# zhaihongjia/SplatLoc

Measured on AMD Instinct MI355X. Metric: fwd+bwd frames/s @1080p, 500k Gaussians, 32 feat-ch; HBM GB/s vs roofline, higher is better.
Workload: dtype f32

## Files before the change

include/splatraster.h:

```cpp
#ifndef SPLATRASTER_H
#define SPLATRASTER_H

#include <stddef.h>
#include <stdint.h>

#ifdef __cplusplus
extern "C" {
#endif

#define SPLATRASTER_ABI_VERSION 20

#define SPLATRASTER_TILE 16

#define SPLATRASTER_OK 0
#define SPLATRASTER_ERR_BAD_ARG 1
#define SPLATRASTER_ERR_HIP 2
#define SPLATRASTER_ERR_UNSUPPORTED 3
#define SPLATRASTER_ERR_OVERFLOW 4
#define SPLATRASTER_WARN_LOOKBACK_STALL 5

typedef struct splatraster_settings {
    int32_t image_height;
    int32_t image_width;
    float tanfovx;
// ... 482 lines not shown
#define SPLATRASTER_STAGE_PAYLOAD 9
#define SPLATRASTER_STAGE_COUNT 10

int splatraster_timing_enable(int on);
int splatraster_timing_select(uint32_t stage_mask);
int splatraster_timing_collect(double* ms, int64_t* counts);


int splatraster_poll_errors(void);
int splatraster_debug_set_spin_limit(uint32_t limit);
int splatraster_debug_set_deterministic(int on);
int splatraster_debug_set_small_panel_max_waves(int waves);
int splatraster_debug_set_split_max_waves(int waves);
int splatraster_debug_set_fwd_team(int mode);
int splatraster_debug_set_payload_stream_min(int64_t instances);
int splatraster_debug_set_front_end(int mode);
int splatraster_debug_set_tile_sort_cap(int keys);
int splatraster_debug_set_sort_fork(int mode);
int splatraster_debug_exp2(int64_t n, const float* x, float* y, void* stream);
int splatraster_debug_poison_lds(uint32_t pattern, void* stream);

const char* splatraster_error_string(int status);
const char* splatraster_last_hip_error(void);
int splatraster_abi_version(void);

#ifdef __cplusplus
}
#endif
#endif
```

splatloc_amd/_native.py:

```python
from __future__ import annotations

import ctypes as C
import os

from . import build as _build

_LIB = None
ABI_VERSION = 20

OK = 0
WARN_LOOKBACK_STALL = 5
_ERR_NAMES = {1: "bad argument", 2: "HIP runtime error", 3: "unsupported configuration",
              4: "tile instance count overflow", 5: "look-back stall (results late, never wrong)"}


class Settings(C.Structure):
    _fields_ = [
        ("image_height", C.c_int32),
        ("image_width", C.c_int32),
        ("tanfovx", C.c_float),
        ("tanfovy", C.c_float),
        ("scale_modifier", C.c_float),
        ("sh_degree", C.c_int32),
        ("sh_coeffs", C.c_int32),
# ... 112 lines not shown
                                            + [_vp] * 14),
    "splatraster_forward_window_geometry_raw": (C.c_int, [C.POINTER(Settings), _i32, C.POINTER(WindowView), _i32, _vp, C.POINTER(RawForward),
                                                          _vp, C.POINTER(_i64), _vp]),
    "splatraster_backward_window_raw": (C.c_int, [C.POINTER(Settings), _i32, C.POINTER(WindowView), _i32, C.POINTER(_i64)]
                                        + [_vp] * 8 + [C.POINTER(RawParams)] + [_vp] * 2),
    "splatraster_get_window_geometry_layout": (C.c_int, [_i32, _i32, C.POINTER(GeometryLayout)]),
    "splatraster_get_window_binning_layout": (C.c_int, [_i32, _i32, _i64, _i32, _i32, _i32, C.POINTER(BinningLayout)]),
    "splatraster_get_window_image_layout": (C.c_int, [_i32, _i32, _i32, C.POINTER(ImageLayout)]),
    "splatraster_debug_set_small_panel_max_waves": (C.c_int, [C.c_int]),
    "splatraster_debug_set_split_max_waves": (C.c_int, [C.c_int]),
    "splatraster_debug_set_fwd_team": (C.c_int, [C.c_int]),
    "splatraster_debug_set_front_end": (C.c_int, [C.c_int]),
    "splatraster_debug_set_tile_sort_cap": (C.c_int, [C.c_int]),
    "splatraster_debug_set_sort_fork": (C.c_int, [C.c_int]),
    "splatraster_debug_set_payload_stream_min": (C.c_int, [C.c_int64]),
    "splatraster_mark_visible": (C.c_int, [_i32, _vp, _vp, _vp, _vp, _vp]),
    "splatraster_get_geometry_layout": (C.c_int, [_i32, C.POINTER(GeometryLayout)]),
    "splatraster_get_binning_layout": (C.c_int, [_i32, _i64, _i32, _i32, _i32, C.POINTER(BinningLayout)]),
    "splatraster_get_image_layout": (C.c_int, [_i32, _i32, C.POINTER(ImageLayout)]),
    "splatraster_sort_tmp_bytes": (_sz, [_i64]),
    "splatraster_sort_pairs_u32": (C.c_int, [_i64, _vp, _vp, _i32, _vp, _vp]),
    "splatraster_timing_enable": (C.c_int, [C.c_int]),
    "splatraster_timing_select": (C.c_int, [C.c_uint32]),
    "splatraster_timing_collect": (C.c_int, [_vp, _vp]),
    "splatknn_workspace_bytes": (_sz, [_i32]),
    "splatknn_dist2": (C.c_int, [_i32, _vp, _vp, _vp, _vp]),
    "splatknn_debug_set_grid_min": (C.c_int, [_i32]),
    "splatraster_grid_encoding_layout": (C.c_int, [_i32] * 5 + [C.c_double, _i32, C.POINTER(GridLayout)]),
    "splatraster_grid_encoding_forward": (C.c_int, [C.POINTER(GridLayout), _i64, _vp, _vp, _vp, _vp]),
    "splatraster_grid_encoding_backward": (C.c_int, [C.POINTER(GridLayout), _i64] + [_vp] * 6),
# ... 84 lines not shown
    got = int(lib.splatraster_abi_version())
    if got != ABI_VERSION:
        raise RuntimeError(f"{path} has ABI version {got}, this binding needs {ABI_VERSION}: stale library, "
                           "rebuild with `python -m splatloc_amd.build --force`")
    for name, (res, args) in SYMBOLS.items():
        fn = getattr(lib, name)
        fn.restype = res
        fn.argtypes = args
    _LIB = lib
    if os.environ.get("SPLATRASTER_SPLIT_MAX_WAVES"):
        lib.splatraster_debug_set_split_max_waves(int(os.environ["SPLATRASTER_SPLIT_MAX_WAVES"]))
    if os.environ.get("SPLATRASTER_FWD_TEAM"):
        lib.splatraster_debug_set_fwd_team(int(os.environ["SPLATRASTER_FWD_TEAM"]))
    if os.environ.get("SPLATRASTER_FRONT_END"):
        lib.splatraster_debug_set_front_end(int(os.environ["SPLATRASTER_FRONT_END"]))
    if os.environ.get("SPLATRASTER_TILE_SORT_CAP"):
        lib.splatraster_debug_set_tile_sort_cap(int(os.environ["SPLATRASTER_TILE_SORT_CAP"]))
    if os.environ.get("SPLATRASTER_SORT_FORK"):
        lib.splatraster_debug_set_sort_fork(int(os.environ["SPLATRASTER_SORT_FORK"]))
    if os.environ.get("SPLATRASTER_SMALL_PANEL_MAX_WAVES"):
        lib.splatraster_debug_set_small_panel_max_waves(int(os.environ["SPLATRASTER_SMALL_PANEL_MAX_WAVES"]))
    return lib


def check(status: int, what: str) -> None:
    if status != OK:
        lib = load()
        detail = lib.splatraster_last_hip_error().decode() if status in (2, 5) else ""
        raise RuntimeError(f"{what} failed: {_ERR_NAMES.get(status, status)} {detail}".strip())

# ... 17 lines not shown
    n = len(STAGES)
    ms = (C.c_double * n)()
    cnt = (C.c_int64 * n)()
    check(load().splatraster_timing_collect(ms, cnt), "timing_collect")
    return {s: (ms[i], cnt[i]) for i, s in enumerate(STAGES)}


def set_deterministic(on: bool) -> None:
    check(load().splatraster_debug_set_deterministic(int(bool(on))), "set_deterministic")


def set_front_end(mode: int) -> None:
    check(load().splatraster_debug_set_front_end(int(mode)), "set_front_end")


def poll_stall() -> bool:
    st = load().splatraster_poll_errors()
    if st == WARN_LOOKBACK_STALL:
        return True
    check(st, "poll_errors")
    return False
```

splatloc_amd/csrc/binning.hip:

```cpp
#include "tile_order.h"
#include "composite_common.h"

namespace sr {

__device__ __forceinline__ int f2i_sat_b(float v)
{
    if (!(v > -1.0e9f)) v = -1.0e9f;
    if (!(v < 1.0e9f)) v = 1.0e9f;
    return (int)v;
}

constexpr int EMIT_BLOCK = 256;
constexpr int EMIT_IPT = 4;
static_assert(EMIT_SPAN == EMIT_BLOCK * EMIT_IPT, "common.h: EMIT_SPAN");

template <typename KeyT>
__global__ void __launch_bounds__(EMIT_BLOCK)
emit_kernel(int64_t R, int P , int Pv , int tiles_per_view, int W, int H,
            const uint32_t* __restrict__ offsets,
            const uint32_t* __restrict__ depth_order, const float4* __restrict__ rec,
            KeyT* __restrict__ keys, uint32_t* __restrict__ vals,
            const uint32_t* __restrict__ span_owner ,
            uint32_t* __restrict__ ranges, uint32_t nranges )
{
// ... 135 lines not shown

int launch_payload(const splatraster_settings& s, int32_t V, int64_t R, const GeomView& g, const BinView& b, hipStream_t stream)
{
    if (R == 0) return SPLATRASTER_OK;
    const int gx = (s.image_width + TILE - 1) / TILE, gy = (s.image_height + TILE - 1) / TILE;
    if (R >= g_payload_stream_min)
        hipLaunchKernelGGL(payload_kernel<true>, dim3((unsigned)((R + 255) / 256)), dim3(256), 0, stream, R, gx, gx * gy, V,
                           b.point_list, b.tile_list, g.rec, b.irec, b.ipack, b.ranges);
    else
        hipLaunchKernelGGL(payload_kernel<false>, dim3((unsigned)((R + 255) / 256)), dim3(256), 0, stream, R, gx, gx * gy, V,
                           b.point_list, b.tile_list, g.rec, b.irec, b.ipack, b.ranges);
    SR_LAUNCH_CHECK();
    return SPLATRASTER_OK;
}

__global__ void __launch_bounds__(ORDER_THREADS)
tile_order_kernel(int T, const uint32_t* __restrict__ ranges, uint32_t* __restrict__ order, uint32_t* __restrict__ nparts)
{
    __shared__ uint32_t s_cnt[ORDER_BUCKETS];
    __shared__ uint32_t s_wsum[ORDER_THREADS / WAVE];
    tile_order_block(T, [&](int i) { return ranges[2 * i + 1] - ranges[2 * i]; }, order, s_cnt, s_wsum, nparts);
}

int launch_tile_order(const splatraster_settings& s, int32_t V, const BinView& b, hipStream_t stream)
{
    const int gx = (s.image_width + TILE - 1) / TILE, gy = (s.image_height + TILE - 1) / TILE;
    if (!use_tile_order(V, gx * gy)) return SPLATRASTER_OK;
    hipLaunchKernelGGL(tile_order_kernel, dim3(1), dim3(ORDER_THREADS), 0, stream, V * gx * gy, b.ranges, b.tile_order, b.nparts);
    SR_LAUNCH_CHECK();
    return SPLATRASTER_OK;
// ... 32 lines not shown
```

splatloc_amd/csrc/capi.hip:

```cpp
#include <string.h>

#include <mutex>
#include <unordered_map>
#include <string>
#include <vector>

#include "common.h"

namespace sr {

static thread_local std::string g_last_error;
static int g_deterministic = 0;
static int g_split_max_waves = SPLIT_MAX_WAVES;
void set_split_max_waves(int waves) { g_split_max_waves = waves < 0 ? SPLIT_MAX_WAVES : (waves > SPLIT_MAX_WAVES ? SPLIT_MAX_WAVES : waves); }
int split_max_waves() { return g_split_max_waves; }

void set_hip_error(hipError_t e, const char* what)
{
    g_last_error = std::string(what) + ": " + hipGetErrorString(e);
}

void set_error_text(const char* text) { g_last_error = text; }

struct StageRec { int stage; hipEvent_t a, b; };
// ... 169 lines not shown
    v.ipack = reinterpret_cast<uint32_t*>(b + L.ipack);
    v.featp = reinterpret_cast<float*>(b + L.featp);
    v.gacc = reinterpret_cast<float*>(b + L.gacc);
    v.pose_acc = reinterpret_cast<float*>(b + L.pose_acc);
    v.ckpt = reinterpret_cast<float*>(b + L.ckpt);
    v.tile_order = reinterpret_cast<uint32_t*>(b + L.tile_order);
    v.nparts = reinterpret_cast<uint32_t*>(b + L.nparts);
    return v;
}

static size_t img_plane_bytes(int32_t W, int32_t H, int32_t V)
{
    return align_up((size_t)W * H * 4 * (size_t)(V > 0 ? V : 1), 256);
}

ImgView img_view(void* base, int32_t W, int32_t H, int32_t V)
{
    char* b = reinterpret_cast<char*>(base);
    ImgView v;
    v.final_T = reinterpret_cast<float*>(b);
    v.n_contrib = reinterpret_cast<uint32_t*>(b + img_plane_bytes(W, H, V));
    return v;
}

static int check_row_index_range(int32_t P, int32_t V, int32_t C)
{
    const uint64_t n = (uint64_t)P * (uint64_t)V;
    if (n > (1ull << 24) || n * (uint64_t)padded_channels(C) >= (1ull << 32)) return SPLATRASTER_ERR_UNSUPPORTED;
    if ((uint64_t)gacc_total_floats(C, (size_t)P, (size_t)V) >= (1ull << 32)) return SPLATRASTER_ERR_UNSUPPORTED;
    return SPLATRASTER_OK;
}

static int check_settings(const splatraster_settings* s)
{
    if (!s) return SPLATRASTER_ERR_BAD_ARG;
    if (s->image_width <= 0 || s->image_height <= 0 || s->channels <= 0) return SPLATRASTER_ERR_BAD_ARG;
// ... 17 lines not shown
        case SPLATRASTER_ERR_HIP: return "HIP runtime error";
        case SPLATRASTER_ERR_UNSUPPORTED: return "unsupported configuration";
        case SPLATRASTER_ERR_OVERFLOW: return "tile instance count overflow";
        case SPLATRASTER_WARN_LOOKBACK_STALL: return "look-back stall (results late, never wrong)";
        default: return "unknown status";
    }
}

const char* splatraster_last_hip_error(void) { return g_last_error.c_str(); }

size_t splatraster_geometry_bytes(int32_t P) { return geom_layout(P, 1).bytes; }
size_t splatraster_binning_bytes(int32_t P, int64_t R, int32_t width, int32_t height, int32_t channels)
{
    return bin_layout(P, 1, R, width, height, channels).bytes;
}
size_t splatraster_image_bytes(int32_t width, int32_t height) { return 2 * img_plane_bytes(width, height, 1); }

size_t splatraster_window_geometry_bytes(int32_t P, int32_t n_views) { return geom_layout(P, n_views).bytes; }
size_t splatraster_window_binning_bytes(int32_t P, int32_t n_views, int64_t R_total, int32_t width, int32_t height,
                                        int32_t channels)
{
    return bin_layout(P, n_views, R_total, width, height, channels).bytes;
}
size_t splatraster_window_image_bytes(int32_t width, int32_t height, int32_t n_views)
{
    return 2 * img_plane_bytes(width, height, n_views);
}

int splatraster_get_geometry_layout(int32_t P, splatraster_geometry_layout* out)
{
    return splatraster_get_window_geometry_layout(P, 1, out);
}
int splatraster_get_window_geometry_layout(int32_t P, int32_t n_views, splatraster_geometry_layout* out)
{
    if (!out || n_views < 1 || n_views > MAX_VIEWS) return SPLATRASTER_ERR_BAD_ARG;
    const GeomLayout L = geom_layout(P, n_views);
    out->rec0 = L.rec0; out->rec1 = L.rec1; out->tiles_touched = L.tiles_touched;
    out->depth_order = L.depth_order; out->offsets = L.offsets; out->rgb = L.rgb;
    out->clamped = L.clamped; out->total = L.bytes;
    return SPLATRASTER_OK;
}
// ... 7 lines not shown
{
    if (!out || n_views < 1 || n_views > MAX_VIEWS) return SPLATRASTER_ERR_BAD_ARG;
    const BinLayout L = bin_layout(P, n_views, R_total, width, height, channels);
    out->point_list = L.valsA; out->tile_list = L.keysA; out->ranges = L.ranges; out->total = L.bytes;
    return SPLATRASTER_OK;
}
int splatraster_get_image_layout(int32_t width, int32_t height, splatraster_image_layout* out)
{
    return splatraster_get_window_image_layout(width, height, 1, out);
}
int splatraster_get_window_image_layout(int32_t width, int32_t height, int32_t n_views, splatraster_image_layout* out)
{
    if (!out || n_views < 1 || n_views > MAX_VIEWS) return SPLATRASTER_ERR_BAD_ARG;
    out->final_T = 0;
    out->n_contrib = img_plane_bytes(width, height, n_views);
    out->total = 2 * img_plane_bytes(width, height, n_views);
    return SPLATRASTER_OK;
}

}

namespace sr {

static int check_window(const splatraster_settings* s, int32_t V, const splatraster_window_view* views)
{
    int st = check_settings(s);
    if (st) return st;
    if (V < 1 || V > MAX_VIEWS || !views) return SPLATRASTER_ERR_BAD_ARG;
    return SPLATRASTER_OK;
}

// ... 14 lines not shown
struct BinScratch { bool on; uint32_t* table; void* scan_tmp; int64_t entries; };

static std::mutex g_front_end_mu;
static std::unordered_map<const void*, bool> g_front_end;
static void front_end_record(const void* geometry, bool on)
{
    std::lock_guard<std::mutex> lk(g_front_end_mu);
    if (g_front_end.size() > (1u << 14)) g_front_end.clear();
    g_front_end[geometry] = on;
}
static int front_end_recorded(const void* geometry)
{
    std::lock_guard<std::mutex> lk(g_front_end_mu);
    auto it = g_front_end.find(geometry);
    return it == g_front_end.end() ? -1 : (it->second ? 1 : 0);
}

static BinScratch bin_scratch(const splatraster_settings& s, int32_t P, int32_t V, void* geometry, bool geometry_stage)
{
    const int gx = (s.image_width + TILE - 1) / TILE, gy = (s.image_height + TILE - 1) / TILE, tiles = gx * gy;
    const GeomLayout L = geom_layout(P, V);
    BinScratch b{};
    if (!geometry || P <= 0) return b;
    const int recorded = geometry_stage ? -1 : front_end_recorded(geometry);
    b.on = recorded >= 0 ? recorded == 1 : use_bins(P, V, gx, gy, L.total - L.sort_keys);
    if (geometry_stage) front_end_record(geometry, b.on);
    if (!b.on) return b;
    char* base = reinterpret_cast<char*>(geometry);
    b.entries = (int64_t)bin_table_entries(P, V, tiles);
    b.table = reinterpret_cast<uint32_t*>(base + L.sort_keys);
// ... 143 lines not shown
        if (st) return st;
        bool in_alt = false;
        {
            StageTimer t(SPLATRASTER_STAGE_TILE_SORT, stream);
            st = keys16 ? sort_pairs_k16(R, k0, v0, k1, v1, bits, b.sort_tmp, stream, &in_alt)
                        : sort_pairs_u32(R, k0, v0, k1, v1, bits, b.sort_tmp, stream, &in_alt);
        }
        if (st) return st;
    }
    if (R == 0) {
        StageTimer t(SPLATRASTER_STAGE_RANGES, stream);
        st = launch_ranges_clear((int32_t)gtiles, b.ranges, stream);
    }
    if (st) return st;
    const float* featp = feat;
    if (R > 0) {
        StageTimer t(SPLATRASTER_STAGE_PAYLOAD, stream);
        if (!bins.on) st = launch_payload(*s, V, R, g, b, stream);
        if (st) return st;
        if (s->channels % 4) {
            st = launch_pad_features(P, s->channels, feat, b.featp, stream);
            featp = b.featp;
        }
    }
    if (st) return st;
    if (!(R > 0 && bins.on)) {
        StageTimer t(SPLATRASTER_STAGE_RANGES, stream);
        st = launch_tile_order(*s, V, b, stream);
    }
    if (st) return st;
    WinOut outs{};
    for (int v = 0; v < V; ++v) {
        outs.color[v] = views[v].out_color;
        outs.depth[v] = views[v].out_depth;
        outs.alpha[v] = views[v].out_alpha;
    }
    StageTimer t(SPLATRASTER_STAGE_COMPOSITE_FWD, stream);
    return launch_composite_fwd(*s, P, V, R, g, b, im, featp, bg, outs, stream);
}

struct BwdRows { GeomView g; BinView b; WinCams cams; WinGrad grads; };
static int window_accumulate(const splatraster_settings* s, int32_t V, const splatraster_window_view* views, int32_t P, int64_t R,
                             const float* bg, const float* colors_precomp, bool sh_colours, void* geometry, const void* binning,
                             const void* image, bool pose, hipStream_t stream, BwdRows* out)
{
    int st = check_row_index_range(P, V, s->channels);
    if (st) return st;
    const int W = s->image_width, H = s->image_height;
    GeomView& g = out->g;
    BinView& b = out->b;
    g = geom_view(geometry, P, V);
// ... 13 lines not shown
    }
    for (int v = 0; v < V; ++v) {
        const int gcv = views[v].color_grad_channels ? views[v].color_grad_channels : C;
        if (gcv != grads.gc) return SPLATRASTER_ERR_BAD_ARG;
        grads.dL_dlast[v] = grads.gc < C ? views[v].dL_dout_last : nullptr;
    }
    for (int v = 0; v < V; ++v) {
        grads.out_color[v] = views[v].out_color;
        grads.out_depth[v] = views[v].out_depth;
        grads.dL_dcolor[v] = views[v].dL_dout_color;
        grads.dL_ddepth[v] = views[v].dL_dout_depth;
        grads.dL_dalpha[v] = views[v].dL_dout_alpha;
        grads.dL_dmeans2D[v] = views[v].dL_dmeans2D;
    }
    const size_t gacc_n = gacc_total_floats(C, (size_t)P, (size_t)V);
    const bool det = g_deterministic != 0;
    long long* gacc64 = nullptr;
    if (det) {
        SR_HIP_CHECK(hipMallocAsync(reinterpret_cast<void**>(&gacc64), sizeof(long long) * gacc_n, stream));
        SR_HIP_CHECK(hipMemsetAsync(gacc64, 0, sizeof(long long) * gacc_n, stream));
    }
    const size_t fill = pose ? (size_t)(reinterpret_cast<char*>(b.pose_acc) - reinterpret_cast<char*>(b.gacc)) + POSE_ACC_BYTES
                             : sizeof(float) * gacc_n;
    SR_HIP_CHECK(hipMemsetAsync(b.gacc, 0, fill, stream));
    grads.bg = bg;
    grads.bg_channels = bg ? s->bg_channels : 0;
    {
        StageTimer t(SPLATRASTER_STAGE_COMPOSITE_BWD, stream);
        if (det) st = launch_composite_bwd(*s, P, V, R, g, b, im, (C % 4) ? b.featp : feat, C, grads, b.gacc, gacc64, 0, stream);
        if (!st) st = launch_composite_bwd(*s, P, V, R, g, b, im, (C % 4) ? b.featp : feat, C, grads, b.gacc, gacc64, 1, stream);
    }
    if (det) {
        if (!st) st = launch_fixed_to_float((int64_t)gacc_n, gacc64, b.gacc, gacc_det_headroom_drop(C, V), stream);
        (void)hipFreeAsync(gacc64, stream);
    }
    return st;
}

static int window_backward(const splatraster_settings* s, int32_t V, const splatraster_window_view* views, int32_t P,
                           int64_t R, const float* bg, const float* means3D, const float* shs, const float* colors_precomp,
                           const float* scales, const float* rotations, const float* cov3D_precomp, void* geometry,
                           const void* binning, const void* image, float* dL_dmeans3D, float* dL_dcolors,
                           float* dL_dopacities, float* dL_dscales, float* dL_drotations, float* dL_dcov3D,
                           float* dL_dshs, float* dL_dviewmatrix, float* dL_dprojmatrix, float* dL_dcampos,
                           hipStream_t stream, const RawBwd* raw = nullptr)
// ... 208 lines not shown
                           nullptr, nullptr, reinterpret_cast<hipStream_t>(stream), &raw);
}

int splatraster_debug_set_small_panel_max_waves(int waves)
{
    set_small_panel_max_waves(waves);
    return SPLATRASTER_OK;
}

int splatraster_debug_set_payload_stream_min(int64_t instances)
{
    sr::set_payload_stream_min(instances);
    return SPLATRASTER_OK;
}

int splatraster_debug_set_front_end(int mode)
{
    set_bin_mode(mode);
    return SPLATRASTER_OK;
}

int splatraster_debug_set_sort_fork(int mode)
{
    set_bin_fork(mode);
    return SPLATRASTER_OK;
}

int splatraster_debug_set_tile_sort_cap(int keys)
{
    set_bin_tile_cap(keys);
// ... 116 lines not shown
```

splatloc_amd/csrc/common.h:

```cpp
#pragma once
#include <hip/hip_runtime.h>
#include <stdint.h>

#include "../../include/splatraster.h"

namespace sr {

constexpr int TILE = SPLATRASTER_TILE;
constexpr int TILE_PIX = TILE * TILE;
constexpr float NEAR_Z = 0.2f;
constexpr float DILATION = 0.3f;
constexpr float ALPHA_MAX = 0.99f;
constexpr float ALPHA_MIN = 1.0f / 255.0f;
constexpr float T_EPS = 0.0001f;
constexpr int WAVE = 64;
constexpr int PREPROCESS_BLOCK = 256;
static inline int preprocess_blocks(int32_t P) { return (P + PREPROCESS_BLOCK - 1) / PREPROCESS_BLOCK; }

void set_hip_error(hipError_t e, const char* what);
void set_error_text(const char* text);

int lookback_error_init();
int lookback_error_poll();
int lookback_set_spin_limit(uint32_t limit);
// ... 66 lines not shown
    uint32_t* keys_tmp;
    uint32_t* vals_tmp;
    void* sort_tmp;
    float4* irec;
    uint32_t* ipack;
    float* featp;
    float* gacc;
    float* pose_acc;
    uint32_t* nparts;
    float* ckpt;
    uint32_t* tile_order;
};
struct ImgView {
    float* final_T;
    uint32_t* n_contrib;
};

GeomView geom_view(void* base, int32_t P, int32_t V);
BinView bin_view(void* base, int32_t P, int32_t V, int64_t R, int32_t W, int32_t H, int32_t C);
ImgView img_view(void* base, int32_t W, int32_t H, int32_t V);

struct RawFwd {
    const float* scaling;
    const float* rotation;
    const float* opacity;
    const float* f_dc;
    const float* extra;
    int E;
    float* scales;
    float* rotations;
// ... 78 lines not shown
constexpr int BIN_BIG_MINE = 1024;
static_assert((size_t)BIN_MAX_TILES * MAX_VIEWS <= (size_t)BIN_BIG_MINE * BIN_BIG_BLOCKS, "every (view, tile) list could be a long one");
void set_bin_mode(int mode);
size_t bin_table_entries(int32_t P, int32_t V, int tiles);
size_t bin_scratch_bytes(int32_t P, int32_t V, int tiles);
bool use_bins(int32_t P, int32_t V, int gx, int gy , size_t scratch_bytes);
int launch_bin_count(const splatraster_settings& s, int32_t P, int32_t V, const GeomView& g, uint32_t* table, void* scan_tmp,
                     hipStream_t stream);
int launch_bin_scatter_sort(const splatraster_settings& s, int32_t P, int32_t V, int64_t R, const GeomView& g,
                            const uint32_t* table, const BinView& b, uint64_t* keys, hipStream_t stream);

int launch_emit(const splatraster_settings& s, int32_t P, int32_t V, int64_t R, const GeomView& g, uint32_t* keys,
                uint32_t* vals, uint32_t* ranges, uint32_t nranges, hipStream_t stream, bool keys16 = false );
int launch_ranges_clear(int32_t tiles, uint32_t* ranges, hipStream_t stream);
int launch_payload(const splatraster_settings& s, int32_t V, int64_t R, const GeomView& g, const BinView& b, hipStream_t stream);
int launch_pad_features(int32_t P, int C, const float* feat, float* featp, hipStream_t stream);
static inline int padded_channels(int C) { return (C + 3) & ~3; }
constexpr int POSE_SETS = 16, POSE_SET_FLOATS = 64;
constexpr size_t POSE_ACC_BYTES = (size_t)POSE_SETS * POSE_SET_FLOATS * sizeof(float) + 256;
__host__ __device__ constexpr int gacc_moment_offset(int C) { return ((C & 15) + 7 <= 16) ? C : ((C + 15) & ~15); }
__host__ __device__ constexpr int gacc_row_floats(int C) { return (gacc_moment_offset(C) + 7 + 15) & ~15; }
__host__ __device__ constexpr int gacc_shared_floats(int C) { return C >= 32 ? (C & ~15) : 0; }
__host__ __device__ constexpr int gacc_view_floats(int C) { return gacc_row_floats(C) - gacc_shared_floats(C); }
__host__ __device__ static inline size_t gacc_total_floats(int C, size_t P, size_t V)
{
    return P * (size_t)gacc_shared_floats(C) + V * P * (size_t)gacc_view_floats(C);
}
struct GaccLayout {
    uint32_t SH, PV;
    uint32_t P;
// ... 19 lines not shown
#define SR_SPLIT_PARTS 4
#endif
constexpr int SPLIT_PARTS = SR_SPLIT_PARTS;
constexpr int SPLIT_PARTS_MAX = 4 * SPLIT_PARTS;
#ifndef SR_SPLIT_LONG
#define SR_SPLIT_LONG 1024
#endif
#ifndef SR_SPLIT_EXTRA_TILES
#define SR_SPLIT_EXTRA_TILES 512
#endif
constexpr int SPLIT_LONG = SR_SPLIT_LONG, SPLIT_EXTRA_TILES = SR_SPLIT_EXTRA_TILES;
static_assert(SPLIT_EXTRA_TILES % 8 == 0, "the extra workgroups use the quadrant id scheme (8 tiles per 32 ids)");
void set_split_max_waves(int waves);
void set_fwd_team(int mode);
void set_payload_stream_min(int64_t instances);
int split_max_waves();
static inline bool split_lists(int C, int V, int tiles) { return C <= 4 && 4 * V * tiles <= split_max_waves(); }
__host__ __device__ static inline uint32_t split_count(uint32_t len, uint32_t rank)
{
    if (rank >= (uint32_t)SPLIT_EXTRA_TILES || len < (uint32_t)SPLIT_LONG) return (uint32_t)SPLIT_PARTS;
    return len < 2u * (uint32_t)SPLIT_LONG ? 2u * (uint32_t)SPLIT_PARTS : (uint32_t)SPLIT_PARTS_MAX;
}
__host__ __device__ static inline uint32_t split_part(uint32_t len, uint32_t np = (uint32_t)SPLIT_PARTS)
{
    return len < (uint32_t)SPLIT_MIN_LIST ? len : ((len / np + 63u) & ~63u);
}

int launch_composite_fwd(const splatraster_settings& s, int32_t P, int32_t V, int64_t R, const GeomView& g, const BinView& b,
                         const ImgView& im, const float* featp , const float* bg,
                         const WinOut& out, hipStream_t stream);
// ... 18 lines not shown
```

splatloc_amd/csrc/composite_fwd.hip:

```cpp
#include <type_traits>

#include "composite_common.h"

#ifndef SR_FWD_FS
#define SR_FWD_FS 24
#endif
#ifndef SR_FWD_STAGE_UNROLL
#define SR_FWD_STAGE_UNROLL 3
#endif

#ifndef SR_FWD_M4
#define SR_FWD_M4 1
#endif
#ifndef SR_FWD_MINW
#define SR_FWD_MINW 4
#endif

namespace sr {


typedef float f32x16 __attribute__((ext_vector_type(16)));
typedef float f32x4 __attribute__((ext_vector_type(4)));

__device__ __forceinline__ void swap_halves(float& x, float& y)
// ... 31 lines not shown
    static constexpr int NM = MFMA ? 32 : 0;
    static constexpr int NV = NC - NM;
    static constexpr int NCP = (NC + 3) & ~3;
    static constexpr bool M4 = SR_FWD_M4 && MFMA && NV > 0 && NV <= 3 && NM + NV < NCP;
    static constexpr int FS = SR_FWD_FS;
};

template <int NC>
__global__ void __launch_bounds__(WAVE, SR_FWD_MINW)
composite_fwd_kernel(int W, int H, int CP4, int c0, int bg_channels, int write_aux, int tiles , int V,
                     int P ,
                     const uint32_t* __restrict__ ranges, const uint32_t* __restrict__ ipack ,
                     const float4* __restrict__ irec, const float4* __restrict__ featp4,
                     const float* __restrict__ bg, WinOut outs,
                     float* __restrict__ final_T_all, uint32_t* __restrict__ n_contrib_all,
                     const uint32_t* __restrict__ tile_order )
{
    static_assert(NC > 4, "narrow layouts have their own kernels");
    using Cfg = FwdCfg<NC>;
    constexpr int NCP = Cfg::NCP, NM = Cfg::NM, NV = Cfg::NV, FS = Cfg::FS;
    constexpr bool MFMA = Cfg::MFMA, M4 = Cfg::M4;
    constexpr int PPR = NCP / 4;
    __shared__ __attribute__((aligned(16))) float4 s_rec0[WAVE + 1];
    __shared__ __attribute__((aligned(16))) float4 s_rec1[WAVE + 1];
    static_assert(FS % 2 == 0, "pairs: an odd round ends below FS, its zeroed row FS - 1 at most");
    __shared__ __attribute__((aligned(16))) float s_feat[FS * NCP];
    __shared__ uint32_t s_cgid[FS];

    int gtile, quad;
    const int gx = (W + TILE - 1) / TILE;
    quadrant_of_block(blockIdx.x, V * tiles, gx, gtile, quad, tile_order);
// ... 131 lines not shown
                    mfma_acc_32x32x2(accA, a32, b0);
                    mfma_acc_32x32x2(accB, a32, b1);
                }
                if (__builtin_amdgcn_ballot_w64(active) == 0) { wave_done = true; break; }
            }
        }
    }

    const size_t plane = (size_t)H * W;
    if constexpr (M4) {
        mfma_drain4(acc4);
#pragma unroll
        for (int ch = 0; ch < NV; ++ch) acc[ch] = acc4[ch];
        D = acc4[3];
    }
    if (MFMA) {
        mfma_drain(accA, accB);
        float TA = T, TB = T;
        swap_halves(TA, TB);
        const int pa = lane & 31, pb = 32 + (lane & 31);
        const int xa = qx + (pa & 7), ya = qy + (pa >> 3), xb = qx + (pb & 7), yb = qy + (pb >> 3);
        const bool ina = xa < W && ya < H, inb = xb < W && yb < H;
#pragma unroll
        for (int r = 0; r < 16; ++r) {
            const int c = c0 + (r & 3) + 8 * (r >> 2) + 4 * (lane >> 5);
            const float bgc = c < bg_channels ? bg[c] : 0.0f;
            if (ina) out_color[(size_t)c * plane + (size_t)ya * W + xa] = accA[r] + TA * bgc;
            if (inb) out_color[(size_t)c * plane + (size_t)yb * W + xb] = accB[r] + TB * bgc;
        }
    }
// ... 7 lines not shown
        if (write_aux) {
            out_depth[pix] = D;
            out_alpha[pix] = 1.0f - T;
            final_T[pix] = T;
            n_contrib[pix] = last;
        }
    }
}

#define SR_FWD_PARAMS                                                                                                        \
    int W, int H, int CP4, int c0, int bg_channels, int write_aux, int tiles , int V, int P ,  \
        const uint32_t *__restrict__ ranges, const uint32_t *__restrict__ ipack ,                  \
        const float4 *__restrict__ irec, const float4 *__restrict__ featp4, const float *__restrict__ bg, WinOut outs,      \
        float *__restrict__ final_T_all, uint32_t *__restrict__ n_contrib_all,                                              \
        float *__restrict__ ckpt_all , \
        const uint32_t *__restrict__ nparts
#define SR_FWD_ARGS W, H, CP4, c0, bg_channels, write_aux, tiles, V, P, ranges, ipack, irec, featp4, bg, outs, final_T_all, n_contrib_all, ckpt_all, nparts

template <int NC>
__device__ __forceinline__ void narrow_quadrant(SR_FWD_PARAMS, int gtile, int quad, int lane, float4* __restrict__ s_rec0,
                                                float4* __restrict__ s_rec1, float4* __restrict__ s_fq)
{
    static_assert(NC >= 1 && NC <= 4, "one 16-byte piece per feature row");
    const int gx = (W + TILE - 1) / TILE;
    const int view = (V == 1) ? 0 : gtile / tiles;
    const int tile = gtile - view * tiles;
    const uint32_t row0 = (uint32_t)view * (uint32_t)P;
    float* __restrict__ out_color = outs.color[view];
    float* __restrict__ out_depth = outs.depth[view];
    float* __restrict__ out_alpha = outs.alpha[view];
    float* __restrict__ final_T = final_T_all + (size_t)view * H * W;
    uint32_t* __restrict__ n_contrib = n_contrib_all + (size_t)view * H * W;
// ... 107 lines not shown
#pragma unroll
                for (int ch = 0; ch < NC; ++ch) sacc[ch] = fmaf(fv1[ch], w1, fmaf(fv0[ch], w0, sacc[ch]));
                sD = fmaf(p1.z, w1, fmaf(p0.z, w0, sD));
            }
            if (__builtin_amdgcn_ballot_w64(active) == 0) { wave_done = true; break; }
        }
    }

    if (part) {
        store_segment(ck_k, false);
#pragma unroll
        for (int ch = 0; ch < NC; ++ch) sacc[ch] = 0.0f;
        sD = 0.0f;
        for (int k = ck_k + 1; k < np; ++k) store_segment(k, false);
    }
    if (inside) {
        const size_t plane = (size_t)H * W;
        const size_t pix = (size_t)py * W + px;
#pragma unroll
        for (int ch = 0; ch < NC; ++ch) {
            const int c = c0 + ch;
            out_color[(size_t)c * plane + pix] = acc[ch] + T * (c < bg_channels ? bg[c] : 0.0f);
        }
        if (write_aux) {
            out_depth[pix] = D;
            out_alpha[pix] = 1.0f - T;
            final_T[pix] = T;
            n_contrib[pix] = last;
        }
    }
// ... 372 lines not shown
{
    hipLaunchKernelGGL(debug_exp2_kernel, dim3((unsigned)((n + 255) / 256)), dim3(256), 0, stream, n, x, y);
    SR_LAUNCH_CHECK();
    return SPLATRASTER_OK;
}

struct FwdLaunch {
    int P, V;
    const WinOut* outs;
    float* ckpt;
    bool team;
};

static int g_fwd_team = -1;
void set_fwd_team(int mode) { g_fwd_team = mode; }

template <int NC>
static int launch_one(const splatraster_settings& s, int c0, int write_aux, const GeomView& g,
                      const BinView& b, const ImgView& im, const float* featp, int feat_stride,
                      const float* bg, const FwdLaunch& L, hipStream_t stream)
{
    (void)g;
    const int gx = (s.image_width + TILE - 1) / TILE, gy = (s.image_height + TILE - 1) / TILE;
    const int tiles = gx * gy;
    const unsigned blocks = quadrant_blocks(L.V * tiles, gx);
    if constexpr (NC <= 4) {
        if (L.team && use_tile_order(L.V, tiles)) {
            hipLaunchKernelGGL(composite_fwd_mixed_kernel<NC>, dim3((unsigned)(L.V * tiles + 4 * TEAM_MAX)), dim3(4 * WAVE), 0, stream,
                               s.image_width, s.image_height, padded_channels(feat_stride) / 4, c0, s.bg_channels, write_aux, tiles, L.V, L.P,
                               b.ranges, b.ipack, b.irec, reinterpret_cast<const float4*>(featp), bg, *L.outs, im.final_T, im.n_contrib,
                               (c0 == 0 && write_aux) ? L.ckpt : nullptr, b.nparts, b.tile_order, g_fwd_team == 2 ? 1 : 0);
        } else {
            hipLaunchKernelGGL(composite_fwd_narrow_kernel<NC>, dim3(blocks), dim3(WAVE), 0, stream, s.image_width,
                               s.image_height, padded_channels(feat_stride) / 4, c0, s.bg_channels, write_aux, tiles, L.V, L.P, b.ranges,
                               b.ipack, b.irec, reinterpret_cast<const float4*>(featp), bg, *L.outs, im.final_T,
                               im.n_contrib, (c0 == 0 && write_aux) ? L.ckpt : nullptr, use_tile_order(L.V, tiles) ? b.nparts : nullptr,
                               use_tile_order(L.V, tiles) ? b.tile_order : nullptr);
        }
    } else {
        hipLaunchKernelGGL(composite_fwd_kernel<NC>, dim3(blocks), dim3(WAVE), 0, stream, s.image_width,
                           s.image_height, padded_channels(feat_stride) / 4, c0, s.bg_channels, write_aux, tiles, L.V, L.P, b.ranges,
                           b.ipack, b.irec, reinterpret_cast<const float4*>(featp), bg, *L.outs, im.final_T,
                           im.n_contrib, use_tile_order(L.V, tiles) ? b.tile_order : nullptr);
    }
    SR_LAUNCH_CHECK();
    return SPLATRASTER_OK;
}

int launch_composite_fwd(const splatraster_settings& s, int32_t P, int32_t V, int64_t R, const GeomView& g, const BinView& b,
                         const ImgView& im, const float* featp, const float* bg, const WinOut& outs, hipStream_t stream)
{
    (void)R;
    const int C = s.channels;
    const int tiles_v = ((s.image_width + TILE - 1) / TILE) * ((s.image_height + TILE - 1) / TILE);
    const bool team = g_fwd_team < 0 ? split_lists(C, V, tiles_v) : (g_fwd_team != 0 && C <= 4);
    const FwdLaunch L{P, V, &outs, split_lists(C, V, tiles_v) ? b.ckpt : nullptr, team};
    int c0 = 0, aux = 1, st = SPLATRASTER_OK;
#define SR_FWD_CASE(N)                                                                              \
    case N:                                                                                         \
        return launch_one<N>(s, 0, 1, g, b, im, featp, C, bg, L, stream);
    switch (C) {
        SR_FWD_CASE(1) SR_FWD_CASE(2) SR_FWD_CASE(3) SR_FWD_CASE(4) SR_FWD_CASE(8) SR_FWD_CASE(16)
        SR_FWD_CASE(32) SR_FWD_CASE(35)
        default: break;
    }
#undef SR_FWD_CASE
    while (c0 < C && st == SPLATRASTER_OK) {
        const int left = C - c0;
        if (left >= 32) { st = launch_one<32>(s, c0, aux, g, b, im, featp, C, bg, L, stream); c0 += 32; }
        else if (left >= 16) { st = launch_one<16>(s, c0, aux, g, b, im, featp, C, bg, L, stream); c0 += 16; }
// ... 13 lines not shown
```

splatloc_amd/introspect.py:

```python
from __future__ import annotations

import ctypes as C

import torch

from . import _native


def _view(buf: torch.Tensor, off: int, count: int, dtype: torch.dtype) -> torch.Tensor:
    nbytes = count * torch.empty((), dtype=dtype).element_size()
    return buf[off:off + nbytes].view(dtype)


def geometry_views(geom: torch.Tensor, P: int) -> dict:
    lib = _native.load()
    L = _native.GeometryLayout()
    _native.check(lib.splatraster_get_geometry_layout(P, C.byref(L)), "geometry_layout")
    return dict(
        rec0=_view(geom, L.rec0, 8 * P, torch.float32).view(P, 8)[:, :4],
        rec1=_view(geom, L.rec0, 8 * P, torch.float32).view(P, 8)[:, 4:],
        tiles_touched=_view(geom, L.tiles_touched, P, torch.int32),
        depth_order=_view(geom, L.depth_order, P, torch.int32) & 0xFFFFFF,
        offsets=_view(geom, L.offsets, P, torch.int32),
        rgb=_view(geom, L.rgb, 3 * P, torch.float32).view(P, 3),
# ... 11 lines not shown
        tile_list=_view(binning, L.tile_list, R, torch.int32),
        ranges=_view(binning, L.ranges, 2 * tiles, torch.int32).view(tiles, 2),
    )


def image_views(img: torch.Tensor, W: int, H: int) -> dict:
    lib = _native.load()
    L = _native.ImageLayout()
    _native.check(lib.splatraster_get_image_layout(W, H, C.byref(L)), "image_layout")
    return dict(
        final_T=_view(img, L.final_T, W * H, torch.float32).view(H, W),
        n_contrib=_view(img, L.n_contrib, W * H, torch.int32).view(H, W),
    )


def forward_buffers(grad_fn):
    from .rasterizer import _saved
    b = _saved(grad_fn)[1]
    return b["geom"], b["binning"], b["img"]


def forward_state(fn_ctx_tensors, P: int, W: int, H: int, R: int) -> dict:
    geom, binning, img = fn_ctx_tensors
    out = {}
    out.update(geometry_views(geom, P))
    out.update(binning_views(binning, P, R, W, H))
    out.update(image_views(img, W, H))
    return out


# ... 28 lines not shown
```

Measured before the change: 773.7.

## Compact per-tile payload lists by culling instances that miss every tile quadrant

Adds a payload kernel that runs one block per tile. It tests each instance against the tile's quadrants and writes only live instances into a compacted irec/ipack, along with compacted ranges. The forward composite records a compacted n_contrib and maps it back to the original index through a back pointer stored in irec.w. The backward pass uses the compacted ranges and counts, so both composites iterate over fewer dead instances. In exchange it adds a separate ranges kernel, a per-tile block-scan payload pass with extra syncs, extra image buffer planes, and a host map that records the mode per binning buffer.

```diff
diff --git a/include/splatraster.h b/include/splatraster.h
--- a/include/splatraster.h
+++ b/include/splatraster.h
@@ -520,6 +520,7 @@
 int splatraster_debug_set_split_max_waves(int waves);
 int splatraster_debug_set_fwd_team(int mode);
 int splatraster_debug_set_payload_stream_min(int64_t instances);
+int splatraster_debug_set_payload_compact(int mode);
 int splatraster_debug_set_front_end(int mode);
 int splatraster_debug_set_tile_sort_cap(int keys);
 int splatraster_debug_set_sort_fork(int mode);
diff --git a/splatloc_amd/_native.py b/splatloc_amd/_native.py
--- a/splatloc_amd/_native.py
+++ b/splatloc_amd/_native.py
@@ -150,6 +150,7 @@
     "splatraster_debug_set_tile_sort_cap": (C.c_int, [C.c_int]),
     "splatraster_debug_set_sort_fork": (C.c_int, [C.c_int]),
     "splatraster_debug_set_payload_stream_min": (C.c_int, [C.c_int64]),
+    "splatraster_debug_set_payload_compact": (C.c_int, [C.c_int]),
     "splatraster_mark_visible": (C.c_int, [_i32, _vp, _vp, _vp, _vp, _vp]),
     "splatraster_get_geometry_layout": (C.c_int, [_i32, C.POINTER(GeometryLayout)]),
     "splatraster_get_binning_layout": (C.c_int, [_i32, _i64, _i32, _i32, _i32, C.POINTER(BinningLayout)]),
@@ -264,6 +265,8 @@
         lib.splatraster_debug_set_fwd_team(int(os.environ["SPLATRASTER_FWD_TEAM"]))
     if os.environ.get("SPLATRASTER_FRONT_END"):
         lib.splatraster_debug_set_front_end(int(os.environ["SPLATRASTER_FRONT_END"]))
+    if os.environ.get("SPLATRASTER_PAYLOAD_COMPACT"):
+        lib.splatraster_debug_set_payload_compact(int(os.environ["SPLATRASTER_PAYLOAD_COMPACT"]))
     if os.environ.get("SPLATRASTER_TILE_SORT_CAP"):
         lib.splatraster_debug_set_tile_sort_cap(int(os.environ["SPLATRASTER_TILE_SORT_CAP"]))
     if os.environ.get("SPLATRASTER_SORT_FORK"):
@@ -311,6 +314,10 @@
     check(load().splatraster_debug_set_front_end(int(mode)), "set_front_end")
 
 
+def set_payload_compact(mode: int) -> None:
+    check(load().splatraster_debug_set_payload_compact(int(mode)), "set_payload_compact")
+
+
 def poll_stall() -> bool:
     st = load().splatraster_poll_errors()
     if st == WARN_LOOKBACK_STALL:
diff --git a/splatloc_amd/csrc/binning.hip b/splatloc_amd/csrc/binning.hip
--- a/splatloc_amd/csrc/binning.hip
+++ b/splatloc_amd/csrc/binning.hip
@@ -173,6 +173,94 @@
     return SPLATRASTER_OK;
 }
 
+__global__ void __launch_bounds__(256)
+ranges_kernel(int64_t R, const uint32_t* __restrict__ tile_list, uint32_t* __restrict__ ranges)
+{
+    const int64_t j = (int64_t)blockIdx.x * blockDim.x + threadIdx.x;
+    if (j >= R) return;
+    const uint32_t t = tile_list[j];
+    if (j == 0 || tile_list[j - 1] != t) ranges[2 * t] = (uint32_t)j;
+    if (j == R - 1 || tile_list[j + 1] != t) ranges[2 * t + 1] = (uint32_t)(j + 1);
+}
+
+template <bool NT>
+__global__ void __launch_bounds__(256)
+payload_tile_kernel(int gx, int tiles_per_view, const uint32_t* __restrict__ ranges, const uint32_t* __restrict__ point_list,
+                    const float4* __restrict__ rec, float4* __restrict__ irec, uint32_t* __restrict__ ipack,
+                    uint32_t* __restrict__ cranges)
+{
+    __shared__ uint32_t s_live[4];
+    const uint32_t gt = blockIdx.x;
+    const uint32_t beg = ranges[2 * gt], end = ranges[2 * gt + 1];
+    const uint32_t tl = gt % (uint32_t)tiles_per_view;
+    const uint32_t ty = tl / (uint32_t)gx, tx = tl - ty * (uint32_t)gx;
+    const float ox = (float)(tx * TILE), oy = (float)(ty * TILE);
+    const int lane = threadIdx.x & (WAVE - 1);
+    const int wave = __builtin_amdgcn_readfirstlane((int)(threadIdx.x >> 6));
+    const uint64_t lt_mask = (lane == 0) ? 0ull : (~0ull >> (WAVE - lane));
+    uint32_t running = 0;
+#pragma unroll 1
+    for (uint32_t base = beg; base < end; base += 256u) {
+        const uint32_t j = base + threadIdx.x;
+        uint32_t g = 0u, mask = 0u;
+        float4 a0 = make_float4(0.f, 0.f, 0.f, 0.f), a1 = a0;
+        if (j < end) {
+            g = point_list[j];
+            a0 = rec[2 * (size_t)g];
+            a1 = rec[2 * (size_t)g + 1];
+            mask = quadrant_reach_mask(a0, a1, ox, oy);
+        }
+        const bool live = mask != 0u;
+        const uint64_t ballot = __builtin_amdgcn_ballot_w64(live);
+        if (lane == 0) s_live[wave] = (uint32_t)__popcll(ballot);
+        __syncthreads();
+        const uint32_t n0 = s_live[0], n1 = s_live[1], n2 = s_live[2], n3 = s_live[3];
+        __syncthreads();
+        const uint32_t before = (wave > 0 ? n0 : 0u) + (wave > 1 ? n1 : 0u) + (wave > 2 ? n2 : 0u);
+        if (live) {
+            const size_t pos = (size_t)beg + running + before + (uint32_t)__popcll(ballot & lt_mask);
+            const float4 c1 = payload_conic(a1);
+            const float back = __uint_as_float(j - beg + 1u);
+            const uint32_t m = g | (mask << 24);
+            if (NT) {
+                typedef float f32x4_t __attribute__((ext_vector_type(4)));
+                f32x4_t* out = reinterpret_cast<f32x4_t*>(irec) + 2 * pos;
+                __builtin_nontemporal_store((f32x4_t){a0.x, a0.y, a0.z, back}, out);
+                __builtin_nontemporal_store((f32x4_t){c1.x, c1.y, c1.z, c1.w}, out + 1);
+                __builtin_nontemporal_store(m, ipack + pos);
+            } else {
+                irec[2 * pos] = make_float4(a0.x, a0.y, a0.z, back);
+                irec[2 * pos + 1] = c1;
+                ipack[pos] = m;
+            }
+        }
+        running += n0 + n1 + n2 + n3;
+    }
+    if (threadIdx.x == 0) {
+        cranges[2 * gt] = beg;
+        cranges[2 * gt + 1] = beg + running;
+    }
+}
+
+int launch_payload_compact(const splatraster_settings& s, int32_t V, int64_t R, const GeomView& g, const BinView& b,
+                           uint32_t* cranges, hipStream_t stream)
+{
+    const int gx = (s.image_width + TILE - 1) / TILE, gy = (s.image_height + TILE - 1) / TILE;
+    const unsigned lists = (unsigned)(V * gx * gy);
+    if (R > 0) {
+        hipLaunchKernelGGL(ranges_kernel, dim3((unsigned)((R + 255) / 256)), dim3(256), 0, stream, R, b.tile_list, b.ranges);
+        SR_LAUNCH_CHECK();
+    }
+    if (R >= g_payload_stream_min)
+        hipLaunchKernelGGL(payload_tile_kernel<true>, dim3(lists), dim3(256), 0, stream, gx, gx * gy, b.ranges, b.point_list, g.rec,
+                           b.irec, b.ipack, cranges);
+    else
+        hipLaunchKernelGGL(payload_tile_kernel<false>, dim3(lists), dim3(256), 0, stream, gx, gx * gy, b.ranges, b.point_list, g.rec,
+                           b.irec, b.ipack, cranges);
+    SR_LAUNCH_CHECK();
+    return SPLATRASTER_OK;
+}
+
 __global__ void __launch_bounds__(ORDER_THREADS)
 tile_order_kernel(int T, const uint32_t* __restrict__ ranges, uint32_t* __restrict__ order, uint32_t* __restrict__ nparts)
 {
diff --git a/splatloc_amd/csrc/capi.hip b/splatloc_amd/csrc/capi.hip
--- a/splatloc_amd/csrc/capi.hip
+++ b/splatloc_amd/csrc/capi.hip
@@ -207,12 +207,20 @@
     return align_up((size_t)W * H * 4 * (size_t)(V > 0 ? V : 1), 256);
 }
 
+static size_t img_cranges_bytes(int32_t W, int32_t H, int32_t V)
+{
+    return align_up(8 * (size_t)((W + TILE - 1) / TILE) * (size_t)((H + TILE - 1) / TILE) * (size_t)(V > 0 ? V : 1), 256);
+}
+static size_t img_bytes(int32_t W, int32_t H, int32_t V) { return 3 * img_plane_bytes(W, H, V) + img_cranges_bytes(W, H, V); }
+
 ImgView img_view(void* base, int32_t W, int32_t H, int32_t V)
 {
     char* b = reinterpret_cast<char*>(base);
     ImgView v;
     v.final_T = reinterpret_cast<float*>(b);
     v.n_contrib = reinterpret_cast<uint32_t*>(b + img_plane_bytes(W, H, V));
+    v.n_contrib_c = reinterpret_cast<uint32_t*>(b + 2 * img_plane_bytes(W, H, V));
+    v.cranges = reinterpret_cast<uint32_t*>(b + 3 * img_plane_bytes(W, H, V));
     return v;
 }
 
@@ -260,7 +268,7 @@
 {
     return bin_layout(P, 1, R, width, height, channels).bytes;
 }
-size_t splatraster_image_bytes(int32_t width, int32_t height) { return 2 * img_plane_bytes(width, height, 1); }
+size_t splatraster_image_bytes(int32_t width, int32_t height) { return img_bytes(width, height, 1); }
 
 size_t splatraster_window_geometry_bytes(int32_t P, int32_t n_views) { return geom_layout(P, n_views).bytes; }
 size_t splatraster_window_binning_bytes(int32_t P, int32_t n_views, int64_t R_total, int32_t width, int32_t height,
@@ -270,7 +278,7 @@
 }
 size_t splatraster_window_image_bytes(int32_t width, int32_t height, int32_t n_views)
 {
-    return 2 * img_plane_bytes(width, height, n_views);
+    return img_bytes(width, height, n_views);
 }
 
 int splatraster_get_geometry_layout(int32_t P, splatraster_geometry_layout* out)
@@ -308,7 +316,7 @@
     if (!out || n_views < 1 || n_views > MAX_VIEWS) return SPLATRASTER_ERR_BAD_ARG;
     out->final_T = 0;
     out->n_contrib = img_plane_bytes(width, height, n_views);
-    out->total = 2 * img_plane_bytes(width, height, n_views);
+    out->total = img_bytes(width, height, n_views);
     return SPLATRASTER_OK;
 }
 
@@ -353,6 +361,26 @@
     std::lock_guard<std::mutex> lk(g_front_end_mu);
     auto it = g_front_end.find(geometry);
     return it == g_front_end.end() ? -1 : (it->second ? 1 : 0);
+}
+
+static int g_payload_compact = -1;
+static bool payload_compact(const splatraster_settings& s, int32_t V, int64_t R, bool binned)
+{
+    const int tiles = ((s.image_width + TILE - 1) / TILE) * ((s.image_height + TILE - 1) / TILE);
+    return g_payload_compact != 0 && R > 0 && !binned && !split_lists(s.channels, V, tiles) && !fwd_team_launch(s.channels, V, tiles);
+}
+static std::unordered_map<const void*, bool> g_compact;
+static void compact_record(const void* binning, bool on)
+{
+    std::lock_guard<std::mutex> lk(g_front_end_mu);
+    if (g_compact.size() > (1u << 14)) g_compact.clear();
+    g_compact[binning] = on;
+}
+static int compact_recorded(const void* binning)
+{
+    std::lock_guard<std::mutex> lk(g_front_end_mu);
+    auto it = g_compact.find(binning);
+    return it == g_compact.end() ? -1 : (it->second ? 1 : 0);
 }
 
 static BinScratch bin_scratch(const splatraster_settings& s, int32_t P, int32_t V, void* geometry, bool geometry_stage)
@@ -526,9 +554,12 @@
     }
     if (st) return st;
     const float* featp = feat;
+    const bool compact = payload_compact(*s, V, R, bins.on);
+    compact_record(binning, compact);
     if (R > 0) {
         StageTimer t(SPLATRASTER_STAGE_PAYLOAD, stream);
-        if (!bins.on) st = launch_payload(*s, V, R, g, b, stream);
+        if (compact) st = launch_payload_compact(*s, V, R, g, b, im.cranges, stream);
+        else if (!bins.on) st = launch_payload(*s, V, R, g, b, stream);
         if (st) return st;
         if (s->channels % 4) {
             st = launch_pad_features(P, s->channels, feat, b.featp, stream);
@@ -547,6 +578,8 @@
         outs.depth[v] = views[v].out_depth;
         outs.alpha[v] = views[v].out_alpha;
     }
+    if (compact) b.ranges = im.cranges;
+    else im.n_contrib_c = nullptr;
     StageTimer t(SPLATRASTER_STAGE_COMPOSITE_FWD, stream);
     return launch_composite_fwd(*s, P, V, R, g, b, im, featp, bg, outs, stream);
 }
@@ -590,6 +623,10 @@
         grads.dL_dmeans2D[v] = views[v].dL_dmeans2D;
     }
     const size_t gacc_n = gacc_total_floats(C, (size_t)P, (size_t)V);
+    const int rec_c = compact_recorded(binning);
+    const bool compact = rec_c >= 0 ? rec_c == 1 : payload_compact(*s, V, R, bin_scratch(*s, P, V, geometry, false).on);
+    BinView bw = b;
+    if (compact) { bw.ranges = im.cranges; im.n_contrib = im.n_contrib_c; }
     const bool det = g_deterministic != 0;
     long long* gacc64 = nullptr;
     if (det) {
@@ -603,8 +640,8 @@
     grads.bg_channels = bg ? s->bg_channels : 0;
     {
         StageTimer t(SPLATRASTER_STAGE_COMPOSITE_BWD, stream);
-        if (det) st = launch_composite_bwd(*s, P, V, R, g, b, im, (C % 4) ? b.featp : feat, C, grads, b.gacc, gacc64, 0, stream);
-        if (!st) st = launch_composite_bwd(*s, P, V, R, g, b, im, (C % 4) ? b.featp : feat, C, grads, b.gacc, gacc64, 1, stream);
+        if (det) st = launch_composite_bwd(*s, P, V, R, g, bw, im, (C % 4) ? b.featp : feat, C, grads, b.gacc, gacc64, 0, stream);
+        if (!st) st = launch_composite_bwd(*s, P, V, R, g, bw, im, (C % 4) ? b.featp : feat, C, grads, b.gacc, gacc64, 1, stream);
     }
     if (det) {
         if (!st) st = launch_fixed_to_float((int64_t)gacc_n, gacc64, b.gacc, gacc_det_headroom_drop(C, V), stream);
@@ -843,6 +880,12 @@
     return SPLATRASTER_OK;
 }
 
+int splatraster_debug_set_payload_compact(int mode)
+{
+    g_payload_compact = mode < 0 ? -1 : (mode ? 1 : 0);
+    return SPLATRASTER_OK;
+}
+
 int splatraster_debug_set_front_end(int mode)
 {
     set_bin_mode(mode);
diff --git a/splatloc_amd/csrc/common.h b/splatloc_amd/csrc/common.h
--- a/splatloc_amd/csrc/common.h
+++ b/splatloc_amd/csrc/common.h
@@ -104,6 +104,8 @@
 struct ImgView {
     float* final_T;
     uint32_t* n_contrib;
+    uint32_t* n_contrib_c;
+    uint32_t* cranges;
 };
 
 GeomView geom_view(void* base, int32_t P, int32_t V);
@@ -212,6 +214,8 @@
                 uint32_t* vals, uint32_t* ranges, uint32_t nranges, hipStream_t stream, bool keys16 = false );
 int launch_ranges_clear(int32_t tiles, uint32_t* ranges, hipStream_t stream);
 int launch_payload(const splatraster_settings& s, int32_t V, int64_t R, const GeomView& g, const BinView& b, hipStream_t stream);
+int launch_payload_compact(const splatraster_settings& s, int32_t V, int64_t R, const GeomView& g, const BinView& b,
+                           uint32_t* cranges, hipStream_t stream);
 int launch_pad_features(int32_t P, int C, const float* feat, float* featp, hipStream_t stream);
 static inline int padded_channels(int C) { return (C + 3) & ~3; }
 constexpr int POSE_SETS = 16, POSE_SET_FLOATS = 64;
@@ -261,6 +265,7 @@
 void set_split_max_waves(int waves);
 void set_fwd_team(int mode);
 void set_payload_stream_min(int64_t instances);
+bool fwd_team_launch(int C, int V, int tiles);
 int split_max_waves();
 static inline bool split_lists(int C, int V, int tiles) { return C <= 4 && 4 * V * tiles <= split_max_waves(); }
 __host__ __device__ static inline uint32_t split_count(uint32_t len, uint32_t rank)
diff --git a/splatloc_amd/csrc/composite_fwd.hip b/splatloc_amd/csrc/composite_fwd.hip
--- a/splatloc_amd/csrc/composite_fwd.hip
+++ b/splatloc_amd/csrc/composite_fwd.hip
@@ -69,7 +69,8 @@
                      const float4* __restrict__ irec, const float4* __restrict__ featp4,
                      const float* __restrict__ bg, WinOut outs,
                      float* __restrict__ final_T_all, uint32_t* __restrict__ n_contrib_all,
-                     const uint32_t* __restrict__ tile_order )
+                     const uint32_t* __restrict__ tile_order ,
+                     uint32_t* __restrict__ n_contrib_c_all )
 {
     static_assert(NC > 4, "narrow layouts have their own kernels");
     using Cfg = FwdCfg<NC>;
@@ -231,6 +232,10 @@
         for (int ch = 0; ch < NV; ++ch) acc[ch] = acc4[ch];
         D = acc4[3];
     }
+    if (n_contrib_c_all != nullptr && write_aux && inside) {
+        (n_contrib_c_all + (size_t)view * H * W)[(size_t)py * W + px] = last;
+        if (last) last = __float_as_uint(irec[2 * (size_t)(beg + last - 1u)].w);
+    }
     if (MFMA) {
         mfma_drain(accA, accB);
         float TA = T, TB = T;
@@ -268,8 +273,9 @@
         const float4 *__restrict__ irec, const float4 *__restrict__ featp4, const float *__restrict__ bg, WinOut outs,      \
         float *__restrict__ final_T_all, uint32_t *__restrict__ n_contrib_all,                                              \
         float *__restrict__ ckpt_all , \
-        const uint32_t *__restrict__ nparts
-#define SR_FWD_ARGS W, H, CP4, c0, bg_channels, write_aux, tiles, V, P, ranges, ipack, irec, featp4, bg, outs, final_T_all, n_contrib_all, ckpt_all, nparts
+        const uint32_t *__restrict__ nparts , \
+        uint32_t *__restrict__ n_contrib_c_all
+#define SR_FWD_ARGS W, H, CP4, c0, bg_channels, write_aux, tiles, V, P, ranges, ipack, irec, featp4, bg, outs, final_T_all, n_contrib_all, ckpt_all, nparts, n_contrib_c_all
 
 template <int NC>
 __device__ __forceinline__ void narrow_quadrant(SR_FWD_PARAMS, int gtile, int quad, int lane, float4* __restrict__ s_rec0,
@@ -407,6 +413,10 @@
         sD = 0.0f;
         for (int k = ck_k + 1; k < np; ++k) store_segment(k, false);
     }
+    if (n_contrib_c_all != nullptr && write_aux && inside) {
+        (n_contrib_c_all + (size_t)view * H * W)[(size_t)py * W + px] = last;
+        if (last) last = __float_as_uint(irec[2 * (size_t)(beg + last - 1u)].w);
+    }
     if (inside) {
         const size_t plane = (size_t)H * W;
         const size_t pix = (size_t)py * W + px;
@@ -809,6 +819,7 @@
 
 static int g_fwd_team = -1;
 void set_fwd_team(int mode) { g_fwd_team = mode; }
+bool fwd_team_launch(int C, int V, int tiles) { return g_fwd_team < 0 ? split_lists(C, V, tiles) : (g_fwd_team != 0 && C <= 4); }
 
 template <int NC>
 static int launch_one(const splatraster_settings& s, int c0, int write_aux, const GeomView& g,
@@ -824,19 +835,20 @@
             hipLaunchKernelGGL(composite_fwd_mixed_kernel<NC>, dim3((unsigned)(L.V * tiles + 4 * TEAM_MAX)), dim3(4 * WAVE), 0, stream,
                                s.image_width, s.image_height, padded_channels(feat_stride) / 4, c0, s.bg_channels, write_aux, tiles, L.V, L.P,
                                b.ranges, b.ipack, b.irec, reinterpret_cast<const float4*>(featp), bg, *L.outs, im.final_T, im.n_contrib,
-                               (c0 == 0 && write_aux) ? L.ckpt : nullptr, b.nparts, b.tile_order, g_fwd_team == 2 ? 1 : 0);
+                               (c0 == 0 && write_aux) ? L.ckpt : nullptr, b.nparts, (uint32_t*)nullptr ,
+                               b.tile_order, g_fwd_team == 2 ? 1 : 0);
         } else {
             hipLaunchKernelGGL(composite_fwd_narrow_kernel<NC>, dim3(blocks), dim3(WAVE), 0, stream, s.image_width,
                                s.image_height, padded_channels(feat_stride) / 4, c0, s.bg_channels, write_aux, tiles, L.V, L.P, b.ranges,
                                b.ipack, b.irec, reinterpret_cast<const float4*>(featp), bg, *L.outs, im.final_T,
                                im.n_contrib, (c0 == 0 && write_aux) ? L.ckpt : nullptr, use_tile_order(L.V, tiles) ? b.nparts : nullptr,
-                               use_tile_order(L.V, tiles) ? b.tile_order : nullptr);
+                               im.n_contrib_c, use_tile_order(L.V, tiles) ? b.tile_order : nullptr);
         }
     } else {
         hipLaunchKernelGGL(composite_fwd_kernel<NC>, dim3(blocks), dim3(WAVE), 0, stream, s.image_width,
                            s.image_height, padded_channels(feat_stride) / 4, c0, s.bg_channels, write_aux, tiles, L.V, L.P, b.ranges,
                            b.ipack, b.irec, reinterpret_cast<const float4*>(featp), bg, *L.outs, im.final_T,
-                           im.n_contrib, use_tile_order(L.V, tiles) ? b.tile_order : nullptr);
+                           im.n_contrib, use_tile_order(L.V, tiles) ? b.tile_order : nullptr, im.n_contrib_c);
     }
     SR_LAUNCH_CHECK();
     return SPLATRASTER_OK;
@@ -848,7 +860,8 @@
     (void)R;
     const int C = s.channels;
     const int tiles_v = ((s.image_width + TILE - 1) / TILE) * ((s.image_height + TILE - 1) / TILE);
-    const bool team = g_fwd_team < 0 ? split_lists(C, V, tiles_v) : (g_fwd_team != 0 && C <= 4);
+    const bool team = fwd_team_launch(C, V, tiles_v);
+    if (im.n_contrib_c != nullptr && (team || split_lists(C, V, tiles_v))) return SPLATRASTER_ERR_BAD_ARG;
     const FwdLaunch L{P, V, &outs, split_lists(C, V, tiles_v) ? b.ckpt : nullptr, team};
     int c0 = 0, aux = 1, st = SPLATRASTER_OK;
 #define SR_FWD_CASE(N)                                                                              \
diff --git a/splatloc_amd/introspect.py b/splatloc_amd/introspect.py
--- a/splatloc_amd/introspect.py
+++ b/splatloc_amd/introspect.py
@@ -49,6 +49,32 @@
     )
 
 
+def payload_state(fn_ctx_tensors, R: int, W: int, H: int, V: int = 1, compact: bool = True) -> dict:
+    lib = _native.load()
+    _geom, binning, img = fn_ctx_tensors
+    BL, IL = _native.BinningLayout(), _native.ImageLayout()
+    _native.check(lib.splatraster_get_window_binning_layout(1, V, R, W, H, 4, C.byref(BL)), "window_binning_layout")
+    _native.check(lib.splatraster_get_window_image_layout(W, H, V, C.byref(IL)), "window_image_layout")
+    al = lambda b: (b + 255) // 256 * 256
+    tiles = V * ((W + 15) // 16) * ((H + 15) // 16)
+    n = max(int(R), 1)
+    irec_off = BL.ranges + al(8 * tiles) + al(lib.splatraster_sort_tmp_bytes(n) - 2 * al(4 * n))
+    irec = _view(binning, irec_off, 8 * int(R), torch.float32).view(int(R), 8)
+    ipack = _view(binning, irec_off + al(32 * n), int(R), torch.int32)
+    out = {}
+    if compact:
+        plane = IL.n_contrib
+        cr = _view(img, 3 * plane, 2 * tiles, torch.int32).view(tiles, 2).long()
+        lens = cr[:, 1] - cr[:, 0]
+        first = torch.cumsum(lens, 0) - lens
+        idx = torch.repeat_interleave(cr[:, 0] - first, lens) + torch.arange(int(lens.sum()), device=lens.device)
+        irec, ipack = irec[idx], ipack[idx]
+        out.update(cranges=cr.int(), n_contrib_c=_view(img, 2 * plane, V * W * H, torch.int32).view(V, H, W),
+                   back=irec[:, 3].contiguous().view(torch.int32))
+    out.update(irec=irec, ids=ipack & 0xFFFFFF, imask=(ipack >> 24) & 0xF)
+    return out
+
+
 def forward_buffers(grad_fn):
     from .rasterizer import _saved
     b = _saved(grad_fn)[1]
```

Result: faster. 789.3, median of 6 (+2.0%).
